# ShenhanQian/GaussianAvatars

Hardware: AMD Instinct MI355X
Metric: frames/sec fwd+bwd @100k SH-3 splats 802x550 (higher is better)
Workload: dtype f32; 1 GPU; BASELINE configs[2]: 100000 mesh-bound SH-3 splats (synthetic stand-in for media/306), 802x550 (HxW), select_mesh_by_timestep + render + L1-vs-white + backward, no optimiser step; splats=100000, width=550, height=802, sh_degree=3, scene=ellipsoid, splat_order=morton (io.spatial_sort: the loaders' default), num_rendered=2322054, num_binned=1851307, tile_culling=True, binding=fused, parallelism=one process, one GPU, 300 frames in turn; no collective

## Files before the change

### gaussianavatars_amd/csrc/gsr_backward.hip

```cpp
#include "gsr_device.h"

#include <hip/amd_detail/amd_hip_unsafe_atomics.h>

namespace gsr {

__device__ __forceinline__ float swap32_add(float a, float b)
{
    const auto r = __builtin_amdgcn_permlane32_swap(__float_as_uint(a), __float_as_uint(b), false, false);
    return __uint_as_float(r[0]) + __uint_as_float(r[1]);
}
__device__ __forceinline__ float swap16_add(float a, float b)
{
    const auto r = __builtin_amdgcn_permlane16_swap(__float_as_uint(a), __float_as_uint(b), false, false);
    return __uint_as_float(r[0]) + __uint_as_float(r[1]);
}
__device__ __forceinline__ float bank_merge(float keep, float take, const int bank_mask_sel)
{
    return bank_mask_sel == 0xA
               ? __int_as_float(__builtin_amdgcn_update_dpp(__float_as_int(keep), __float_as_int(take), 0xE4, 0xf, 0xA, false))
               : __int_as_float(__builtin_amdgcn_update_dpp(__float_as_int(keep), __float_as_int(take), 0xE4, 0xf, 0xC, false));
}
__device__ __forceinline__ float row_sum4(float a, float b, float c, float d)
{
    a += dpp_f<0x141, 0xf>(a);
// ... 354 lines not shown
    const float fqx0 = (float)qx0, fqy0 = (float)qy0;

    for (;;) {
        const int lo = hi - CH;
        const int j = hi - 1 - lane;
        const bool valid = lane < CH && j < nq;
        const uint32_t idx = qp[valid ? j : nq - 1];
        const float4 r0 = grec[3 * (size_t)idx + 0], r1 = grec[3 * (size_t)idx + 1], r2 = grec[3 * (size_t)idx + 2];
        const float xq = r0.x - fqx0, yq = r0.y - fqy0;
        const float cA = r0.z, cB = r0.w, cC = r1.x;
        const float op = valid ? r2.z : 0.f;
        const float cr = r1.z, cgn = r1.w, cb = r2.x;
        const int jrec = valid ? j : 0x7fffffff;
        const unsigned long long act = __ballot(last_pix > lo);
        const bool more = lo > seg_lo;
        f2 a0 = {0.f, 0.f}, a1 = a0, a2 = a0, a3 = a0, a4 = a0, a5 = a0, a6 = a0, a7 = a0, a8 = a0;

        for (int r = 0; r < 8; ++r) {
            const uint32_t rm = (uint32_t)(act >> (8 * r)) & 0xFFu;
            if (!rm) continue;
            const float dy = yq - (float)r;
            const float Bdy = cB * dy, Cdy2 = (cC * dy) * dy;
#ifndef GSR_EXP_NO_ROW_SUMS
            f2 rs0 = {0.f, 0.f}, rs1 = rs0, rs2 = rs0;
#endif
#pragma unroll
            for (int h = 0; h < 2; ++h) {
                if (!((rm >> (4 * h)) & 0xFu)) continue;
                const f4* tp = reinterpret_cast<const f4*>(tab + (r * 4 + 2 * h) * 12);
                f4 t[2][3];
#pragma unroll
                for (int e = 0; e < 2; ++e)
#pragma unroll
                    for (int k = 0; k < 3; ++k) t[e][k] = tp[3 * e + k];
                f2 dx[2], a0m[2], al[2], rv[2], R[2], Tj[2], cg[2], aT[2], Pw[2];
#pragma unroll
                for (int e = 0; e < 2; ++e) {
                    const float c0 = (float)(4 * h + 2 * e);
                    dx[e] = f2{xq - c0, xq - (c0 + 1.0f)};
                    const f2 pw = (cA * dx[e] + Bdy) * dx[e] + Cdy2;
                    const f2 G = {__builtin_amdgcn_exp2f(pw.x), __builtin_amdgcn_exp2f(pw.y)};
                    const f2 araw = op * G;
                    const int l0 = __float_as_int(t[e][2].z), l1 = __float_as_int(t[e][2].w);
#ifdef GSR_EXP_HI_TEST
                    a0m[e].x = (l0 > jrec && pw.x <= 0.0f && araw.x >= 1.0f / 255.0f) ? araw.x : 0.0f;
                    a0m[e].y = (l1 > jrec && pw.y <= 0.0f && araw.y >= 1.0f / 255.0f) ? araw.y : 0.0f;
#else
                    a0m[e].x = (l0 > jrec && araw.x >= 1.0f / 255.0f) ? araw.x : 0.0f;
                    a0m[e].y = (l1 > jrec && araw.y >= 1.0f / 255.0f) ? araw.y : 0.0f;
#endif
                    al[e] = f2{__builtin_fminf(0.99f, a0m[e].x), __builtin_fminf(0.99f, a0m[e].y)};
                    const f2 om = 1.0f - al[e];
                    rv[e] = f2{__builtin_amdgcn_rcpf(om.x), __builtin_amdgcn_rcpf(om.y)};
                    R[e] = rv[e];
                }
#ifndef GSR_EXP_RP_NOSCAN
                GSR_SCAN4("v_mul_f32_dpp", R[0].x, R[0].y, R[1].x, R[1].y);
#endif
#pragma unroll
                for (int e = 0; e < 2; ++e) {
                    const f2 Te = {t[e][0].x, t[e][0].y};
                    const f2 g0 = {t[e][1].x, t[e][1].y}, g1 = {t[e][1].z, t[e][1].w}, g2 = {t[e][2].x, t[e][2].y};
                    Tj[e] = Te * R[e];
                    cg[e] = cr * g0 + (cgn * g1 + cb * g2);
                    aT[e] = al[e] * Tj[e];
                    Pw[e] = aT[e] * cg[e];
                }
#ifndef GSR_EXP_RP_NOSCAN
                GSR_SCAN4("v_add_f32_dpp", Pw[0].x, Pw[0].y, Pw[1].x, Pw[1].y);
#endif
#pragma unroll
                for (int e = 0; e < 2; ++e) {
                    const f2 Sx = {t[e][0].z, t[e][0].w};
                    const f2 g0 = {t[e][1].x, t[e][1].y}, g1 = {t[e][1].z, t[e][1].w}, g2 = {t[e][2].x, t[e][2].y};
                    const f2 dLda = ((Tj[e] * cg[e] - Pw[e]) - Sx) * rv[e];
                    const f2 tq = a0m[e] * dLda;
                    a0 += aT[e] * g0;
                    a1 += aT[e] * g1;
                    a2 += aT[e] * g2;
#ifndef GSR_EXP_NO_ROW_SUMS
                    const f2 ax = tq * dx[e];
                    rs0 += tq;
                    rs1 += ax;
                    rs2 += ax * dx[e];
#else
                    const f2 ax = tq * dx[e], ay = tq * dy;
                    a3 += ax;
                    a4 += ay;
                    a5 += ax * dx[e];
                    a6 += ax * dy;
                    a7 += ay * dy;
                    a8 += tq;
#endif
                    if (more) {
                        const float T0 = __int_as_float(__builtin_amdgcn_readlane(__float_as_int(Tj[e].x), CH - 1));
                        const float T1 = __int_as_float(__builtin_amdgcn_readlane(__float_as_int(Tj[e].y), CH - 1));
                        const float S0 = __int_as_float(__builtin_amdgcn_readlane(__float_as_int(Pw[e].x), CH - 1)) + Sx.x;
                        const float S1 = __int_as_float(__builtin_amdgcn_readlane(__float_as_int(Pw[e].y), CH - 1)) + Sx.y;
                        if (lane == 0) {
                            float* up = tab + (r * 4 + 2 * h + e) * 12;
                            up[0] = T0; up[1] = T1; up[2] = S0; up[3] = S1;
                        }
                    }
                }
            }
#ifndef GSR_EXP_NO_ROW_SUMS
            a3 += rs1;
            a4 += rs0 * dy;
            a5 += rs2;
            a6 += rs1 * dy;
            a7 += rs0 * (dy * dy);
            a8 += rs0;
#endif
        }
#ifndef GSR_EXP_RP_NOATOMIC
        {
            const float v[9] = {a0.x + a0.y, a1.x + a1.y, a2.x + a2.y, a3.x + a3.y, a4.x + a4.y, a5.x + a5.y, a6.x + a6.y, a7.x + a7.y, a8.x + a8.y};
#pragma unroll
            for (int c = 0; c < 9; ++c) xs[9 * lane + c] = v[c];
#pragma unroll
            for (int i = 0; i < (CH + 6) / 7; ++i) {
                const int rl7 = (lane * 7282) >> 16;
                const int c = lane - 9 * rl7;
                const int rl = 7 * i + rl7;
                const float val = xs[63 * i + lane];
                const uint32_t rid = (uint32_t)__builtin_amdgcn_ds_bpermute(rl << 2, (int)idx);
                const bool live = lane < 63 && rl < CH && (hi - 1 - rl) < nq;
#ifdef GSR_EXP_RP_PLAINSTORE
                if (live && val == 12345.678f) acc[(size_t)GSR_ACC_STRIDE * rid + c] = val;
#else
                if (live && val != 0.f) unsafeAtomicAdd(acc + (size_t)GSR_ACC_STRIDE * rid + c, val);
#endif
            }
        }
#endif
        if (!more) break;
        hi = lo;
    }
    }
}

template __global__ void k_render_bwd_rp<1>(Settings, const uint32_t*, const uint32_t*, const float4*, const uint32_t*, const float*, const uint32_t*, const float*, float*, const float*,
                                             const float4*, int, unsigned long long, const unsigned long long*, const uint32_t*);
template __global__ void k_render_bwd_rp<2>(Settings, const uint32_t*, const uint32_t*, const float4*, const uint32_t*, const float*, const uint32_t*, const float*, float*, const float*,
                                             const float4*, int, unsigned long long, const unsigned long long*, const uint32_t*);
template __global__ void k_render_bwd_rp<4>(Settings, const uint32_t*, const uint32_t*, const float4*, const uint32_t*, const float*, const uint32_t*, const float*, float*, const float*,
                                             const float4*, int, unsigned long long, const unsigned long long*, const uint32_t*);


__global__ __launch_bounds__(GSR_PREBWD_ROWS) void k_preprocess_bwd(Settings s, PreBwdArgs a)
{
    const int i = blockIdx.x * blockDim.x + threadIdx.x;
    const int M = a.M;
    __shared__ float sh_lds[GSR_PREBWD_ROWS * GSR_SH_MAX_STRIDE];
    const bool sh_staged = !a.use_precomp_color && a.dL_dsh != nullptr && M <= 16;
    const int first = blockIdx.x * GSR_PREBWD_ROWS, rows = min(GSR_PREBWD_ROWS, a.P - first);
    const int sh_stride = sh_row_stride(M);
    if (sh_staged) {
        if (a.shs_rest) {
            sh_rows_load<GSR_PREBWD_ROWS>(sh_lds, a.shs, first, rows, 3, sh_stride, 0, (int)threadIdx.x);
            sh_rows_load<GSR_PREBWD_ROWS>(sh_lds, a.shs_rest, first, rows, 3 * (M - 1), sh_stride, 3, (int)threadIdx.x);
        } else {
            sh_rows_load<GSR_PREBWD_ROWS>(sh_lds, a.shs, first, rows, 3 * M, sh_stride, 0, (int)threadIdx.x);
        }
        __syncthreads();
    }
    if (i < a.P) {
    float dmean[3] = {0.f, 0.f, 0.f};
    float gcov[6] = {0.f, 0.f, 0.f, 0.f, 0.f, 0.f};
    float dscale[3] = {0.f, 0.f, 0.f};
    float drot[4] = {0.f, 0.f, 0.f, 0.f};
    float gcol[3] = {0.f, 0.f, 0.f};
    float g2x = 0.f, g2y = 0.f, gop = 0.f;
    const bool vis = a.radii[i] > 0;
    float* gsh = a.dL_dsh ? (sh_staged ? sh_lds + (int)threadIdx.x * sh_row_stride(M) : a.dL_dsh + (size_t)3 * M * i) : nullptr;

    if (vis) {
        float4 q0, q1, q2;
        if (s.deterministic) {
            long long* ai = a.acc64 + (size_t)GSR_ACC64_STRIDE * i;
            const int ex = __float_as_int(a.grec[3 * (size_t)i + 2].y), back = gmax_exponent(*a.gmax) - GSR_FIXED_BITS;
            float f[9];
#pragma unroll
            for (int k = 0; k < 9; ++k) { f[k] = __builtin_ldexpf((float)ai[k], back + ((k >= 5 && k <= 7) ? (ex >> 8) : (ex & 0xFF))); ai[k] = 0ll; }
            q0 = make_float4(f[0], f[1], f[2], f[3]); q1 = make_float4(f[4], f[5], f[6], f[7]); q2 = make_float4(f[8], 0.f, 0.f, 0.f);
        } else {
            float4* ac4 = (float4*)(a.acc + (size_t)GSR_ACC_STRIDE * i);
            q0 = ac4[0]; q1 = ac4[1]; q2 = ac4[2];
            const float4 z = make_float4(0.f, 0.f, 0.f, 0.f);
            ac4[0] = z; ac4[1] = z; ac4[2] = z;
        }
        gcol[0] = q0.x; gcol[1] = q0.y; gcol[2] = q0.z;
        g2x = -0.5f * (float)s.W * q0.w; g2y = -0.5f * (float)s.H * q1.x;
        const float gA = -0.5f * q1.y, gB = -0.5f * q1.z, gC = -0.5f * q1.w;
        gop = q2.x;
        const float* vm = s.viewmatrix;
        const float* proj = s.projmatrix;
        const int W = s.W, H = s.H;
        const float fx = (float)W / (2.0f * s.tanfovx), fy = (float)H / (2.0f * s.tanfovy);
        float mx = a.means3D[3 * i], my = a.means3D[3 * i + 1], mz = a.means3D[3 * i + 2];
        if (a.bound.binding) {
            const long long bface = bound_face(a.bound, i);
            float w[3];
            bindm::world_xyz(a.bound.fR + 9 * bface, a.bound.fs[bface], a.bound.fc + 3 * bface, mx, my, mz, w);
            mx = w[0]; my = w[1]; mz = w[2];
        }
        const float* c6 = a.cov3D + 6 * i;

        if (!a.use_precomp_color) {
            float shr[48];
            {
                const float* row = sh_staged ? sh_lds + (int)threadIdx.x * sh_row_stride(M) : a.shs + (size_t)3 * M * i;
#pragma unroll
                for (int k = 0; k < 48; ++k) shr[k] = k < 3 * M ? row[k] : 0.f;
            }
            const float* sh = shr;
            const int deg = s.sh_degree;
            const float d0 = mx - s.campos[0], d1 = my - s.campos[1], d2 = mz - s.campos[2];
            const float sum2 = d0 * d0 + d1 * d1 + d2 * d2;
            const float inv_len = 1.0f / sqrtf(sum2);
            const float x = d0 * inv_len, y = d1 * inv_len, z = d2 * inv_len;
            const uint32_t cl = a.clamped[i];
            float ddir[3] = {0.f, 0.f, 0.f};
            const float xx = x * x, yy = y * y, zz = z * z, xy_ = x * y, yz = y * z, xz = x * z;
            const int ncoef = (deg + 1) * (deg + 1);
#pragma unroll
            for (int c = 0; c < 3; ++c) {
                const float g = ((cl >> c) & 1u) ? 0.f : gcol[c];
                float dxs = 0.f, dys = 0.f, dzs = 0.f;
                gsh[0 + c] = kC0 * g;
                if (deg > 0) {
                    gsh[3 + c] = -kC1 * y * g;
                    gsh[6 + c] = kC1 * z * g;
                    gsh[9 + c] = -kC1 * x * g;
                    dxs = -kC1 * sh[9 + c];
                    dys = -kC1 * sh[3 + c];
                    dzs = kC1 * sh[6 + c];
                    if (deg > 1) {
                        gsh[12 + c] = kC2_0 * xy_ * g;
                        gsh[15 + c] = kC2_1 * yz * g;
                        gsh[18 + c] = kC2_2 * (2.f * zz - xx - yy) * g;
                        gsh[21 + c] = kC2_3 * xz * g;
                        gsh[24 + c] = kC2_4 * (xx - yy) * g;
                        dxs += kC2_0 * y * sh[12 + c] + kC2_2 * 2.f * -x * sh[18 + c] + kC2_3 * z * sh[21 + c] + kC2_4 * 2.f * x * sh[24 + c];
                        dys += kC2_0 * x * sh[12 + c] + kC2_1 * z * sh[15 + c] + kC2_2 * 2.f * -y * sh[18 + c] + kC2_4 * 2.f * -y * sh[24 + c];
                        dzs += kC2_1 * y * sh[15 + c] + kC2_2 * 2.f * 2.f * z * sh[18 + c] + kC2_3 * x * sh[21 + c];
                        if (deg > 2) {
                            gsh[27 + c] = kC3_0 * y * (3.f * xx - yy) * g;
                            gsh[30 + c] = kC3_1 * xy_ * z * g;
                            gsh[33 + c] = kC3_2 * y * (4.f * zz - xx - yy) * g;
                            gsh[36 + c] = kC3_3 * z * (2.f * zz - 3.f * xx - 3.f * yy) * g;
                            gsh[39 + c] = kC3_4 * x * (4.f * zz - xx - yy) * g;
                            gsh[42 + c] = kC3_5 * z * (xx - yy) * g;
                            gsh[45 + c] = kC3_6 * x * (xx - 3.f * yy) * g;
                            dxs += kC3_0 * sh[27 + c] * 3.f * 2.f * xy_ + kC3_1 * sh[30 + c] * yz + kC3_2 * sh[33 + c] * -2.f * xy_ +
                                   kC3_3 * sh[36 + c] * -3.f * 2.f * xz + kC3_4 * sh[39 + c] * (-3.f * xx + 4.f * zz - yy) +
                                   kC3_5 * sh[42 + c] * 2.f * xz + kC3_6 * sh[45 + c] * 3.f * (xx - yy);
                            dys += kC3_0 * sh[27 + c] * 3.f * (xx - yy) + kC3_1 * sh[30 + c] * xz +
                                   kC3_2 * sh[33 + c] * (-3.f * yy + 4.f * zz - xx) + kC3_3 * sh[36 + c] * -3.f * 2.f * yz +
                                   kC3_4 * sh[39 + c] * -2.f * xy_ + kC3_5 * sh[42 + c] * -2.f * yz + kC3_6 * sh[45 + c] * -3.f * 2.f * xy_;
                            dzs += kC3_1 * sh[30 + c] * xy_ + kC3_2 * sh[33 + c] * 4.f * 2.f * yz +
                                   kC3_3 * sh[36 + c] * 3.f * (2.f * zz - xx - yy) + kC3_4 * sh[39 + c] * 4.f * 2.f * xz +
                                   kC3_5 * sh[42 + c] * (xx - yy);
                        }
                    }
                }
                ddir[0] += dxs * g;
                ddir[1] += dys * g;
                ddir[2] += dzs * g;
            }
            for (int k = 3 * ncoef; k < 3 * M; ++k) gsh[k] = 0.f;
            const float invsum32 = 1.0f / sqrtf(sum2 * sum2 * sum2);
            dmean[0] += ((sum2 - d0 * d0) * ddir[0] - d1 * d0 * ddir[1] - d2 * d0 * ddir[2]) * invsum32;
            dmean[1] += (-d0 * d1 * ddir[0] + (sum2 - d1 * d1) * ddir[1] - d2 * d1 * ddir[2]) * invsum32;
            dmean[2] += (-d0 * d2 * ddir[0] - d1 * d2 * ddir[1] + (sum2 - d2 * d2) * ddir[2]) * invsum32;
        }

        float t0 = vm[0] * mx + vm[4] * my + vm[8] * mz + vm[12];
        float t1 = vm[1] * mx + vm[5] * my + vm[9] * mz + vm[13];
        const float t2 = vm[2] * mx + vm[6] * my + vm[10] * mz + vm[14];
        const float limx = 1.3f * s.tanfovx, limy = 1.3f * s.tanfovy;
        const float txtz = t0 / t2, tytz = t1 / t2;
        t0 = sel_min(limx, sel_max(-limx, txtz)) * t2;
        t1 = sel_min(limy, sel_max(-limy, tytz)) * t2;
        const float x_grad_mul = (txtz < -limx || txtz > limx) ? 0.f : 1.f;
        const float y_grad_mul = (tytz < -limy || tytz > limy) ? 0.f : 1.f;
        const float J00 = fx / t2, J02 = -(fx * t0) / (t2 * t2), J11 = fy / t2, J12 = -(fy * t1) / (t2 * t2);
        float A[2][3];
#pragma unroll
        for (int j = 0; j < 3; ++j) {
            A[0][j] = J00 * vm[4 * j + 0] + J02 * vm[4 * j + 2];
            A[1][j] = J11 * vm[4 * j + 1] + J12 * vm[4 * j + 2];
        }
        const float V[3][3] = {{c6[0], c6[1], c6[2]}, {c6[1], c6[3], c6[4]}, {c6[2], c6[4], c6[5]}};
        float AV[2][3];
#pragma unroll
        for (int r = 0; r < 2; ++r)
#pragma unroll
            for (int j = 0; j < 3; ++j) AV[r][j] = A[r][0] * V[0][j] + A[r][1] * V[1][j] + A[r][2] * V[2][j];
        const float ca = AV[0][0] * A[0][0] + AV[0][1] * A[0][1] + AV[0][2] * A[0][2] + 0.3f;
        const float cb = AV[0][0] * A[1][0] + AV[0][1] * A[1][1] + AV[0][2] * A[1][2];
        const float cc = AV[1][0] * A[1][0] + AV[1][1] * A[1][1] + AV[1][2] * A[1][2] + 0.3f;
        const float denom = ca * cc - cb * cb;
        if (s.fast_blend) {
            const float det_inv = 1.f / denom;
            const float kA = cc * det_inv, kB = -cb * det_inv, kC = ca * det_inv;
            g2x = -0.5f * (float)s.W * (kA * q0.w + kB * q1.x);
            g2y = -0.5f * (float)s.H * (kC * q1.x + kB * q0.w);
            const float opac = a.grec[3 * (size_t)i + 2].z;
            gop = opac > 0.f ? q2.x / opac : 0.f;
        }
        const float denom2inv = 1.0f / ((denom * denom) + 0.0000001f);
        float dL_da = 0.f, dL_db = 0.f, dL_dc = 0.f;
        if (denom2inv != 0.f) {
            dL_da = denom2inv * (-cc * cc * gA + 2.f * cb * cc * gB + (denom - ca * cc) * gC);
            dL_dc = denom2inv * (-ca * ca * gC + 2.f * ca * cb * gB + (denom - ca * cc) * gA);
            dL_db = denom2inv * 2.f * (cb * cc * gA - (denom + 2.f * cb * cb) * gB + ca * cb * gC);
            gcov[0] = A[0][0] * A[0][0] * dL_da + A[0][0] * A[1][0] * dL_db + A[1][0] * A[1][0] * dL_dc;
            gcov[3] = A[0][1] * A[0][1] * dL_da + A[0][1] * A[1][1] * dL_db + A[1][1] * A[1][1] * dL_dc;
            gcov[5] = A[0][2] * A[0][2] * dL_da + A[0][2] * A[1][2] * dL_db + A[1][2] * A[1][2] * dL_dc;
            gcov[1] = 2.f * A[0][0] * A[0][1] * dL_da + (A[0][0] * A[1][1] + A[0][1] * A[1][0]) * dL_db + 2.f * A[1][0] * A[1][1] * dL_dc;
            gcov[2] = 2.f * A[0][0] * A[0][2] * dL_da + (A[0][0] * A[1][2] + A[0][2] * A[1][0]) * dL_db + 2.f * A[1][0] * A[1][2] * dL_dc;
            gcov[4] = 2.f * A[0][2] * A[0][1] * dL_da + (A[0][1] * A[1][2] + A[0][2] * A[1][1]) * dL_db + 2.f * A[1][1] * A[1][2] * dL_dc;
        }
        float dA[2][3];
#pragma unroll
        for (int j = 0; j < 3; ++j) {
            const float a0v = A[0][0] * V[j][0] + A[0][1] * V[j][1] + A[0][2] * V[j][2];
            const float a1v = A[1][0] * V[j][0] + A[1][1] * V[j][1] + A[1][2] * V[j][2];
            dA[0][j] = 2.f * a0v * dL_da + a1v * dL_db;
            dA[1][j] = 2.f * a1v * dL_dc + a0v * dL_db;
        }
        const float dJ00 = vm[0] * dA[0][0] + vm[4] * dA[0][1] + vm[8] * dA[0][2];
        const float dJ02 = vm[2] * dA[0][0] + vm[6] * dA[0][1] + vm[10] * dA[0][2];
        const float dJ11 = vm[1] * dA[1][0] + vm[5] * dA[1][1] + vm[9] * dA[1][2];
        const float dJ12 = vm[2] * dA[1][0] + vm[6] * dA[1][1] + vm[10] * dA[1][2];
        const float tz = 1.f / t2, tz2 = tz * tz, tz3 = tz2 * tz;
        const float dtx = x_grad_mul * -fx * tz2 * dJ02;
        const float dty = y_grad_mul * -fy * tz2 * dJ12;
        const float dtz = -fx * tz2 * dJ00 - fy * tz2 * dJ11 + (2.f * fx * t0) * tz3 * dJ02 + (2.f * fy * t1) * tz3 * dJ12;
        dmean[0] += vm[0] * dtx + vm[1] * dty + vm[2] * dtz;
        dmean[1] += vm[4] * dtx + vm[5] * dty + vm[6] * dtz;
        dmean[2] += vm[8] * dtx + vm[9] * dty + vm[10] * dtz;

        const float hw = proj[3] * mx + proj[7] * my + proj[11] * mz + proj[15];
        const float m_w = 1.0f / (hw + 0.0000001f);
        const float mul1 = (proj[0] * mx + proj[4] * my + proj[8] * mz + proj[12]) * m_w * m_w;
        const float mul2 = (proj[1] * mx + proj[5] * my + proj[9] * mz + proj[13]) * m_w * m_w;
        dmean[0] += (proj[0] * m_w - proj[3] * mul1) * g2x + (proj[1] * m_w - proj[3] * mul2) * g2y;
        dmean[1] += (proj[4] * m_w - proj[7] * mul1) * g2x + (proj[5] * m_w - proj[7] * mul2) * g2y;
        dmean[2] += (proj[8] * m_w - proj[11] * mul1) * g2x + (proj[9] * m_w - proj[11] * mul2) * g2y;

        if (!a.use_precomp_cov) {
            float4 q = reinterpret_cast<const float4*>(a.rotations)[i];
            float ws[3] = {a.scales[3 * i], a.scales[3 * i + 1], a.scales[3 * i + 2]};
            if (a.bound.binding) {
                const long long bface = bound_face(a.bound, i);
                q = bindm::world_rotation(reinterpret_cast<const float4*>(a.bound.fq)[bface], q);
                const float bscale = a.bound.fs[bface];
#pragma unroll
                for (int k = 0; k < 3; ++k) ws[k] = bindm::world_scaling(ws[k], bscale);
            } else if (a.bound.leaves) {
                q = bindm::unit_rotation(q);
#pragma unroll
                for (int k = 0; k < 3; ++k) ws[k] = bindm::world_scaling(ws[k], 1.f);
            }
            const float r = q.x, x = q.y, y = q.z, z = q.w;
            float R[3][3];
            R[0][0] = 1.f - 2.f * (y * y + z * z);
            R[0][1] = 2.f * (x * y - r * z);
            R[0][2] = 2.f * (x * z + r * y);
            R[1][0] = 2.f * (x * y + r * z);
            R[1][1] = 1.f - 2.f * (x * x + z * z);
            R[1][2] = 2.f * (y * z - r * x);
            R[2][0] = 2.f * (x * z - r * y);
            R[2][1] = 2.f * (y * z + r * x);
            R[2][2] = 1.f - 2.f * (x * x + y * y);
            const float mod = s.scale_modifier;
            const float sc[3] = {mod * ws[0], mod * ws[1], mod * ws[2]};
            const float gS[3][3] = {{gcov[0], 0.5f * gcov[1], 0.5f * gcov[2]},
                                    {0.5f * gcov[1], gcov[3], 0.5f * gcov[4]},
                                    {0.5f * gcov[2], 0.5f * gcov[4], gcov[5]}};
            float dR[3][3];
#pragma unroll
            for (int k = 0; k < 3; ++k) {
                float dMk[3];
#pragma unroll
                for (int j = 0; j < 3; ++j)
                    dMk[j] = 2.0f * sc[k] * (R[0][k] * gS[0][j] + R[1][k] * gS[1][j] + R[2][k] * gS[2][j]);
                dscale[k] = (s.exact_scale_grad ? mod : 1.0f) * (R[0][k] * dMk[0] + R[1][k] * dMk[1] + R[2][k] * dMk[2]);
#pragma unroll
                for (int j = 0; j < 3; ++j) dR[j][k] = sc[k] * dMk[j];
            }
            drot[0] = 2.f * z * (dR[1][0] - dR[0][1]) + 2.f * y * (dR[0][2] - dR[2][0]) + 2.f * x * (dR[2][1] - dR[1][2]);
            drot[1] = 2.f * y * (dR[0][1] + dR[1][0]) + 2.f * z * (dR[0][2] + dR[2][0]) + 2.f * r * (dR[2][1] - dR[1][2]) - 4.f * x * (dR[2][2] + dR[1][1]);
            drot[2] = 2.f * x * (dR[0][1] + dR[1][0]) + 2.f * r * (dR[0][2] - dR[2][0]) + 2.f * z * (dR[1][2] + dR[2][1]) - 4.f * y * (dR[2][2] + dR[0][0]);
            drot[3] = 2.f * r * (dR[1][0] - dR[0][1]) + 2.f * x * (dR[0][2] + dR[2][0]) + 2.f * y * (dR[1][2] + dR[2][1]) - 4.f * z * (dR[1][1] + dR[0][0]);
        }
    } else if (gsh) {
        for (int k = 0; k < 3 * M; ++k) gsh[k] = 0.f;
    }

    if (a.bound.binding) {
        const long long bface = bound_face(a.bound, i);
        float Rf[9];
#pragma unroll
        for (int k = 0; k < 9; ++k) Rf[k] = a.bound.fR[9 * bface + k];
        const float xl[3] = {a.means3D[3 * i], a.means3D[3 * i + 1], a.means3D[3 * i + 2]};
        const float ls[3] = {a.scales ? a.scales[3 * i] : 0.f, a.scales ? a.scales[3 * i + 1] : 0.f, a.scales ? a.scales[3 * i + 2] : 0.f};
        const float4 ql = a.rotations ? reinterpret_cast<const float4*>(a.rotations)[i] : make_float4(1.f, 0.f, 0.f, 0.f);
        float dx[3], dls[3], acc[BINDM_ROW];
        float4 dq;
        bindm::bind_backward(Rf, a.bound.fs[bface], reinterpret_cast<const float4*>(a.bound.fq)[bface], xl, ls, ql, dmean, dscale,
                             make_float4(drot[0], drot[1], drot[2], drot[3]), dx, dls, &dq, acc);
#pragma unroll
        for (int k = 0; k < 3; ++k) { dmean[k] = dx[k]; dscale[k] = dls[k]; }
        drot[0] = dq.x; drot[1] = dq.y; drot[2] = dq.z; drot[3] = dq.w;
        const float o = bindm::sigmoid(a.opacities[i]);
        gop = gop * o * (1.f - o);
        float4* row = reinterpret_cast<float4*>(a.bound.rows + (size_t)BINDM_ROW * a.bound.slot[i]);
#pragma unroll
        for (int k = 0; k < BINDM_ROW / 4; ++k) row[k] = make_float4(acc[4 * k], acc[4 * k + 1], acc[4 * k + 2], acc[4 * k + 3]);
    }
    else if (a.bound.leaves) {
        if (a.scales) {
#pragma unroll
            for (int k = 0; k < 3; ++k) dscale[k] *= bindm::world_scaling(a.scales[3 * i + k], 1.f);
        }
        if (a.rotations) {
            const float4 dq = bindm::unit_rotation_backward(reinterpret_cast<const float4*>(a.rotations)[i], make_float4(drot[0], drot[1], drot[2], drot[3]));
            drot[0] = dq.x; drot[1] = dq.y; drot[2] = dq.z; drot[3] = dq.w;
        }
        const float o = bindm::sigmoid(a.opacities[i]);
        gop = gop * o * (1.f - o);
    }
#pragma unroll
    for (int k = 0; k < 3; ++k) a.dL_dmeans3D[3 * i + k] = dmean[k];
    a.dL_dmeans2D[3 * i + 0] = g2x;
    a.dL_dmeans2D[3 * i + 1] = g2y;
    a.dL_dmeans2D[3 * i + 2] = 0.f;
    if (a.dL_dcolors) {
#pragma unroll
        for (int k = 0; k < 3; ++k) a.dL_dcolors[3 * i + k] = gcol[k];
    }
    a.dL_dopacity[i] = gop;
    if (a.dL_dcov3D) {
#pragma unroll
        for (int k = 0; k < 6; ++k) a.dL_dcov3D[6 * i + k] = gcov[k];
    }
    if (a.dL_dscales) {
#pragma unroll
        for (int k = 0; k < 3; ++k) a.dL_dscales[3 * i + k] = dscale[k];
    }
    if (a.dL_drotations) reinterpret_cast<float4*>(a.dL_drotations)[i] = make_float4(drot[0], drot[1], drot[2], drot[3]);
    }
    if (sh_staged) {
        __syncthreads();
        if (a.shs_rest) {
            sh_rows_store<GSR_PREBWD_ROWS>(sh_lds, a.dL_dsh, first, rows, 3, sh_stride, 0, (int)threadIdx.x);
            sh_rows_store<GSR_PREBWD_ROWS>(sh_lds, a.dL_dsh_rest, first, rows, 3 * (M - 1), sh_stride, 3, (int)threadIdx.x);
        } else {
            sh_rows_store<GSR_PREBWD_ROWS>(sh_lds, a.dL_dsh, first, rows, 3 * M, sh_stride, 0, (int)threadIdx.x);
        }
    }
}

}
```

### gaussianavatars_amd/csrc/gsr_device.h

```cpp
#pragma once
#include <hip/hip_runtime.h>
#include <stdint.h>

#include "../../include/gsr.h"

#define GSR_WAVE 64
#define GSR_TILE_PIX (GSR_BLOCK_X * GSR_BLOCK_Y)
#define GSR_SORT_LDS_KEYS 8192
#define GSR_SORT_XL_KEYS 16384
#define GSR_SORT_SMALL_KEYS 2048
#define GSR_ACC_STRIDE 16
#define GSR_ACC64_STRIDE 10
#define GSR_FIXED_BITS 58
#define GSR_LDS_HIST_TILES 40960
#define GSR_RANK_MAX_BUCKETS 4096
#define GSR_RANK_HIST_TILES (GSR_LDS_HIST_TILES - GSR_RANK_MAX_BUCKETS)
#define GSR_RANK_BANDS 24
#define GSR_RANK_MAX_BANDS 32
#define GSR_RANK_BAND_CHUNK 256
#define GSR_RANK_IDX_BITS 28
#define GSR_RANK_MAX_SPLATS 262144
#define GSR_RANK_TILE_THREADS 512
#define GSR_RANK_WINDOW 4096
#ifndef GSR_RANK_GROUP
// ... 145 lines not shown
    r.px = px; r.py = py; r.A = A; r.B = B; r.C = C;
    r.tau = 0.f; r.nBiC = 0.f; r.nBiA = 0.f;
    if (!(opacity * 255.0f >= 1.0f)) { r.mode = 2; return r; }
    r.tau = logf(255.0f * opacity) * 1.0001f + 1e-3f;
    if (!(A > 0.f && C > 0.f && (A * C - B * B) > 0.f)) { r.mode = 1; return r; }
    r.nBiC = -B / C;
    r.nBiA = -B / A;
    r.mode = 0;
    return r;
}
__device__ __forceinline__ bool rect_reach(const Reach& r, float x0, float y0, float w, float h)
{
    if (r.mode) return r.mode == 1;
    const float a0 = r.px - (x0 + w), a1 = r.px - x0;
    const float b0 = r.py - (y0 + h), b1 = r.py - y0;
    const bool in_x = a0 <= 0.f && a1 >= 0.f, in_y = b0 <= 0.f && b1 >= 0.f;
    if (in_x && in_y) return true;
    const float a = a0 > 0.f ? a0 : a1;
    const float b = b0 > 0.f ? b0 : b1;
    const float dyv = fminf(fmaxf(r.nBiC * a, b0), b1);
    const float qv = 0.5f * (r.A * a * a + 2.f * r.B * a * dyv + r.C * dyv * dyv);
    const float dxh = fminf(fmaxf(r.nBiA * b, a0), a1);
    const float qh = 0.5f * (r.A * dxh * dxh + 2.f * r.B * dxh * b + r.C * b * b);
    const float big = 3.0e38f;
    const float mn = fminf(in_x ? big : qv, in_y ? big : qh);
    return mn * 0.999f - 1e-3f <= r.tau;
}

struct Span {
    float px, py, B, det, twoTA, A, dyr;
    int mode;
};
__device__ __forceinline__ Span span_of(const Reach& r)
{
    Span s;
    s.px = r.px; s.py = r.py; s.B = r.B; s.mode = r.mode;
    s.det = 0.f; s.twoTA = 0.f; s.A = 0.f; s.dyr = 0.f;
    if (r.mode) return s;
    const float T = (r.tau + 1e-3f) / 0.999f;
    s.det = r.A * r.C - r.B * r.B;
    s.twoTA = 2.f * T * r.A;
    s.A = r.A;
    s.dyr = r.nBiC * sqrtf(2.f * T * r.C / s.det);
    if (!(fabsf(s.dyr) < 1e15f && s.twoTA < 1e30f && s.A > 1e-30f && s.A < 1e30f && s.det > 0.f)) s.mode = 1;
    return s;
}
struct Band {
    float dl, dr, Bbl, Bbr;
    int any;
};
__device__ __forceinline__ Band band_of(const Span& s, float y0)
{
    Band e;
    e.dl = e.dr = e.Bbl = e.Bbr = 0.f;
    if (s.mode) { e.any = s.mode == 1 ? 2 : 0; return e; }
    const float b0 = y0 - s.py, b1 = b0 + 7.f;
    const float br = fminf(fmaxf(s.dyr, b0), b1), bl = fminf(fmaxf(-s.dyr, b0), b1);
    e.dr = s.twoTA - s.det * br * br;
    e.dl = s.twoTA - s.det * bl * bl;
    e.Bbr = s.B * br;
    e.Bbl = s.B * bl;
    e.any = (e.dr >= 0.f && e.dl >= 0.f) ? 1 : 0;
    return e;
}
__device__ __forceinline__ bool band_hit(const Band& e, const Span& s, float x0)
{
    const float tl = (s.px - 1e-2f - (x0 + 7.f)) * s.A - e.Bbl;
    const float tr = (x0 - s.px - 1e-2f) * s.A + e.Bbr;
    const bool hit = (tl <= 0.f || e.dl >= tl * tl) && (tr <= 0.f || e.dr >= tr * tr);
    return e.any == 2 || (e.any == 1 && hit);
}

__device__ __forceinline__ void snug_rect(const Reach& r, int& minx, int& miny, int& maxx, int& maxy, uint32_t& n)
{
    if (r.mode == 1 || n == 0) return;
    if (r.mode == 2) { n = 0; return; }
    const float det = r.A * r.C - r.B * r.B;
    const float k = 2.f * r.tau / det;
    const float xr = sqrtf(k * r.C) * 1.001f + 1e-2f, yr = sqrtf(k * r.A) * 1.001f + 1e-2f;
    if (!(xr < 1e9f && yr < 1e9f)) return;
    const float fx = (float)GSR_BLOCK_X, fy = (float)GSR_BLOCK_Y;
    const int lox = (int)ceilf((r.px - xr - (fx - 1.f)) / fx), hix = (int)floorf((r.px + xr) / fx) + 1;
    const int loy = (int)ceilf((r.py - yr - (fy - 1.f)) / fy), hiy = (int)floorf((r.py + yr) / fy) + 1;
    minx = max(minx, lox); maxx = min(maxx, hix);
    miny = max(miny, loy); maxy = min(maxy, hiy);
    n = (maxx > minx && maxy > miny) ? (uint32_t)((maxx - minx) * (maxy - miny)) : 0u;
}

__device__ __forceinline__ uint32_t quadrant_mask_of(const Span& s, float ox, float oy)
{
    uint32_t m = 0u;
#pragma unroll
    for (int by = 0; by < 2; ++by) {
        const float y0 = by ? oy + 8.f : oy;
        const float b0 = y0 - s.py, b1 = b0 + 7.f;
        const float br = fminf(fmaxf(s.dyr, b0), b1), bl = fminf(fmaxf(-s.dyr, b0), b1);
        const float dr = s.twoTA - s.det * br * br;
        const float dl = s.twoTA - s.det * bl * bl;
        const float Bbr = s.B * br;
        const float Bbl = s.B * bl;
        const uint32_t any = (uint32_t)(dr >= 0.f) & (uint32_t)(dl >= 0.f);
#pragma unroll
        for (int bx = 0; bx < 2; ++bx) {
            const float x0 = bx ? ox + 8.f : ox;
            const float tl = (s.px - 1e-2f - (x0 + 7.f)) * s.A - Bbl;
            const float tr = (x0 - s.px - 1e-2f) * s.A + Bbr;
            const uint32_t hit = ((uint32_t)(tl <= 0.f) | (uint32_t)(dl >= tl * tl)) & ((uint32_t)(tr <= 0.f) | (uint32_t)(dr >= tr * tr)) & any;
            m |= hit << (2 * by + bx);
        }
    }
    return s.mode == 1 ? 15u : (s.mode == 2 ? 0u : m);
}
__device__ __forceinline__ uint32_t quadrant_mask(float2 p, float4 co, float ox, float oy)
{
    return quadrant_mask_of(span_of(reach_of(p.x, p.y, co.x, co.y, co.z, co.w)), ox, oy);
}

template <typename F>
__device__ __forceinline__ void for_each_tile(int minx, int miny, int maxx, int maxy, uint32_t n, int gx, F f,
                                              uint32_t payload0, uint32_t payload1)
{
    constexpr uint32_t SMALL = 16;
    if (n > 0 && n <= SMALL) {
        for (int y = miny; y < maxy; ++y)
            for (int x = minx; x < maxx; ++x) f((uint32_t)(y * gx + x), payload0, payload1);
    }
    uint64_t big = __ballot(n > SMALL);
    const int lane = lane_id();
    while (big) {
        const int src = __builtin_ctzll(big);
        big &= big - 1;
        const int bminx = __builtin_amdgcn_readlane(minx, src);
        const int bminy = __builtin_amdgcn_readlane(miny, src);
        const int bmaxx = __builtin_amdgcn_readlane(maxx, src);
        const uint32_t bn = (uint32_t)__builtin_amdgcn_readlane((int)n, src);
        const uint32_t p0 = (uint32_t)__builtin_amdgcn_readlane((int)payload0, src);
        const uint32_t p1 = (uint32_t)__builtin_amdgcn_readlane((int)payload1, src);
        const uint32_t w = (uint32_t)(bmaxx - bminx);
        for (uint32_t k = (uint32_t)lane; k < bn; k += GSR_WAVE) {
            const uint32_t y = (uint32_t)bminy + k / w;
            const uint32_t x = (uint32_t)bminx + k % w;
            f(y * (uint32_t)gx + x, p0, p1);
        }
    }
}

#define GSR_SH_ROWS 256
#ifndef GSR_PREBWD_ROWS
#define GSR_PREBWD_ROWS 208
#endif
#define GSR_SH_MAX_STRIDE 49
__device__ __forceinline__ int sh_row_stride(int M) { return (3 * M) | 1; }

template <int NT = GSR_SH_ROWS>
__device__ __forceinline__ void sh_rows_load(float* __restrict__ lds, const float* __restrict__ src, int first, int rows, int w, int stride,
                                             int col0, int tid)
{
    const int total = rows * w;
    const float* base = src + (size_t)first * w;
    if ((total & 3) == 0 && ((((size_t)first * w) & 3) == 0)) {
        const float4* b4 = reinterpret_cast<const float4*>(base);
        for (int f = tid * 4; f < total; f += NT * 4) {
            const float4 v = b4[f >> 2];
            int r = f / w, c = f - r * w;
            const float e[4] = {v.x, v.y, v.z, v.w};
#pragma unroll
            for (int k = 0; k < 4; ++k) {
                lds[r * stride + col0 + c] = e[k];
                if (++c == w) { c = 0; ++r; }
            }
        }
    } else {
        for (int f = tid; f < total; f += NT) {
            const int r = f / w, c = f - r * w;
            lds[r * stride + col0 + c] = base[f];
        }
    }
}

template <int NT = GSR_SH_ROWS>
__device__ __forceinline__ void sh_rows_store(const float* __restrict__ lds, float* __restrict__ dst, int first, int rows, int w, int stride,
                                              int col0, int tid)
{
    const int total = rows * w;
    float* base = dst + (size_t)first * w;
    if ((total & 3) == 0 && ((((size_t)first * w) & 3) == 0)) {
        float4* b4 = reinterpret_cast<float4*>(base);
        for (int f = tid * 4; f < total; f += NT * 4) {
            int r = f / w, c = f - r * w;
            float e[4];
#pragma unroll
            for (int k = 0; k < 4; ++k) {
                e[k] = lds[r * stride + col0 + c];
                if (++c == w) { c = 0; ++r; }
            }
            b4[f >> 2] = make_float4(e[0], e[1], e[2], e[3]);
        }
    } else {
        for (int f = tid; f < total; f += NT) {
            const int r = f / w, c = f - r * w;
            base[f] = lds[r * stride + col0 + c];
        }
    }
}

#define GSR_STAT_SLOTS 32
struct BinStatSlot {
    uint32_t nvis, dmin_inv, dmax_bits, pad0;
    unsigned long long binned_tiles, rect_total;
    uint32_t pad1[8];
};
struct BinHeader {
    unsigned long long total;
    unsigned long long rect_total;
    uint32_t nvis;
    uint32_t dmin_inv;
    uint32_t dmax_bits;
    uint32_t dmin_bits;
    unsigned long long binned_tiles;
    uint32_t band_total[GSR_RANK_MAX_BANDS];
    uint32_t chunk_imbalance;
    uint32_t pad[21];
    BinStatSlot slot[GSR_STAT_SLOTS];
};
static_assert(sizeof(BinHeader) == 256 + 64 * GSR_STAT_SLOTS, "header layout is part of include/gsr.h");

#define GSR_WALK_MASKS 2
struct QBinArgs {
    int Q, gx;
    uint32_t chunks;
    BinHeader* __restrict__ hdr;
    const float4* __restrict__ brec;
    const uint32_t* __restrict__ order;
    uint32_t* __restrict__ qhist;
    const uint32_t* __restrict__ qprefix;
    const uint32_t* __restrict__ qstart;
    uint32_t* __restrict__ qpos;
    unsigned long long* __restrict__ qmask;
    unsigned long long capacity;
};

struct BoundDev {
    int leaves;
    const void* __restrict__ binding;
    int is64;
    const float* __restrict__ fR;
    const float* __restrict__ fs;
    const float* __restrict__ fc;
    const float* __restrict__ fq;
    const int* __restrict__ slot;
    float* __restrict__ rows;
};
__device__ __forceinline__ long long bound_face(const BoundDev& b, int i)
{
    return b.is64 ? reinterpret_cast<const long long*>(b.binding)[i] : (long long)reinterpret_cast<const int*>(b.binding)[i];
}

struct PreprocessArgs {
    int P, M;
    const float* __restrict__ means3D;
    const float* __restrict__ shs;
    const float* __restrict__ shs_rest;
    const float* __restrict__ colors_precomp;
    const float* __restrict__ opacities;
    const float* __restrict__ scales;
    const float* __restrict__ rotations;
    const float* __restrict__ cov3D_precomp;
    int32_t* __restrict__ radii;
    float* __restrict__ depths;
    float4* __restrict__ grec;
    float* __restrict__ cov3D;
    ushort4* __restrict__ rect;
    uint32_t* __restrict__ tiles_touched;
    uint8_t* __restrict__ clamped;
    uint8_t* __restrict__ visible;
    float4* __restrict__ acc;
    float4* __restrict__ acc64;
    uint32_t* __restrict__ tile_count;
    uint32_t* __restrict__ units;
    unsigned long long* __restrict__ rect_total;
    int tiles;
    float4* __restrict__ brec;
    BinHeader* __restrict__ hdr;
    uint32_t* __restrict__ bcount;
    int nb;
    uint32_t* __restrict__ bcursor;
    uint4* __restrict__ pstat;
    ushort4* __restrict__ srect;
    float4* __restrict__ sspan;
    int cull;
    BoundDev bound;
};

struct PreBwdArgs {
    int P, M;
    const float* __restrict__ means3D;
    const float* __restrict__ shs;
    const float* __restrict__ shs_rest;
    const float* __restrict__ scales;
    const float* __restrict__ rotations;
    const float* __restrict__ cov3D;
    const int32_t* __restrict__ radii;
    const uint8_t* __restrict__ clamped;
    float* __restrict__ acc;
    long long* __restrict__ acc64;
    const uint32_t* __restrict__ gmax;
    const float4* __restrict__ grec;
    int use_precomp_cov, use_precomp_color;
    float* __restrict__ dL_dmeans3D;
    float* __restrict__ dL_dmeans2D;
    float* __restrict__ dL_dsh;
    float* __restrict__ dL_dsh_rest;
    float* __restrict__ dL_dcolors;
    float* __restrict__ dL_dopacity;
    float* __restrict__ dL_dscales;
    float* __restrict__ dL_drotations;
    float* __restrict__ dL_dcov3D;
    BoundDev bound;
    const float* __restrict__ opacities;
};

__global__ void k_preprocess(Settings s, PreprocessArgs a);
__global__ void k_tile_scan(int tiles, const uint32_t* tile_count, uint32_t* tile_start, uint32_t* tile_cursor, uint2* ranges,
                            uint32_t* tile_order, unsigned long long* total_dev, unsigned long long* mailbox, unsigned long long seq, unsigned long long post_capacity);
template <bool CULL>
__global__ void k_count(int P, int gx, int tiles, const ushort4* rect, const uint32_t* tiles_touched, const float4* grec, uint32_t* tile_count,
                        unsigned long long* rect_total, uint32_t* block_hist);
template <bool CULL>
__global__ void k_scatter(int P, int gx, int tiles, const float* depths, const ushort4* rect, const uint32_t* tiles_touched, const float4* grec,
                          const uint32_t* tile_start, uint32_t* tile_cursor, unsigned long long* keys,
                          unsigned long long capacity, const unsigned long long* total_dev, const uint32_t* block_hist);
// ... 131 lines not shown
```

Baseline: 3841 frames/s.

## Hoist per-splat loads ahead of SH staging and coalesce gradient stores via LDS

The preprocess backward kernel now issues every per-splat global load (accumulators, means, covariance, binding face data, rotation, scale, opacity, slot) at kernel entry, before the SH rows are staged into LDS. The SH staging is split into a request phase that keeps float4 loads in registers and a later land phase, so the loads overlap the face-data fetches. The 3-wide per-splat outputs (dmean, means2D grad, dscale, color grad) are written through LDS and emitted as coalesced float4 stores. The aim is to hide memory latency and avoid strided scalar stores, at the cost of higher register pressure, clamped speculative loads for out-of-range threads, and extra barriers.

```diff
diff --git a/gaussianavatars_amd/csrc/gsr_backward.hip b/gaussianavatars_amd/csrc/gsr_backward.hip
--- a/gaussianavatars_amd/csrc/gsr_backward.hip
+++ b/gaussianavatars_amd/csrc/gsr_backward.hip
@@ -530,41 +530,74 @@
 {
     const int i = blockIdx.x * blockDim.x + threadIdx.x;
     const int M = a.M;
-    __shared__ float sh_lds[GSR_PREBWD_ROWS * GSR_SH_MAX_STRIDE];
+    const int ic = min(i, a.P - 1);
+    const bool bound = a.bound.binding != nullptr;
+    const int* bp = reinterpret_cast<const int*>(bound ? a.bound.binding : (const void*)a.radii);
+    const int b_lo = bp[a.bound.is64 && bound ? 2 * (size_t)ic : (size_t)ic], b_hi = bp[a.bound.is64 && bound ? 2 * (size_t)ic + 1 : (size_t)ic];
+    const int radius = a.radii[ic];
+    const float4* ac4r = reinterpret_cast<const float4*>(s.deterministic ? reinterpret_cast<const char*>(a.acc64) : reinterpret_cast<const char*>(a.acc)) +
+                         (size_t)(GSR_ACC_STRIDE / 4) * ic;
+    float4 q0 = ac4r[0], q1 = ac4r[1], q2 = ac4r[2];
+    const float lm[3] = {a.means3D[3 * ic], a.means3D[3 * ic + 1], a.means3D[3 * ic + 2]};
+    const float2* cv = reinterpret_cast<const float2*>(a.cov3D + 6 * (size_t)ic);
+    const float2 cv0 = cv[0], cv1 = cv[1], cv2 = cv[2];
+    const uint32_t cl = (uint32_t)a.clamped[ic];
+    const float4 rec2 = a.grec[3 * (size_t)ic + 2];
+    const float4 ql_raw = *reinterpret_cast<const float4*>(a.rotations ? a.rotations + 4 * (size_t)ic : a.cov3D);
+    const float* lsp = a.scales ? a.scales + 3 * (size_t)ic : a.cov3D;
+    const float ls_raw[3] = {lsp[0], lsp[1], lsp[2]};
+    const float logit = (bound || a.bound.leaves) ? a.opacities[ic] : 0.f;
+    const int slot = (bound ? a.bound.slot : a.radii)[ic];
+    __shared__ __align__(16) float sh_lds[GSR_PREBWD_ROWS * GSR_SH_MAX_STRIDE];
     const bool sh_staged = !a.use_precomp_color && a.dL_dsh != nullptr && M <= 16;
     const int first = blockIdx.x * GSR_PREBWD_ROWS, rows = min(GSR_PREBWD_ROWS, a.P - first);
     const int sh_stride = sh_row_stride(M);
+    const bool sh_split = a.shs_rest != nullptr;
+    ShRowsInFlight<GSR_PREBWD_ROWS, 1> sh_dc;
+    ShRowsInFlight<GSR_PREBWD_ROWS, 12> sh_main;
     if (sh_staged) {
-        if (a.shs_rest) {
-            sh_rows_load<GSR_PREBWD_ROWS>(sh_lds, a.shs, first, rows, 3, sh_stride, 0, (int)threadIdx.x);
-            sh_rows_load<GSR_PREBWD_ROWS>(sh_lds, a.shs_rest, first, rows, 3 * (M - 1), sh_stride, 3, (int)threadIdx.x);
-        } else {
-            sh_rows_load<GSR_PREBWD_ROWS>(sh_lds, a.shs, first, rows, 3 * M, sh_stride, 0, (int)threadIdx.x);
-        }
+        if (sh_split) sh_dc.request(a.shs, first, rows, 3, (int)threadIdx.x);
+        sh_main.request(sh_split ? a.shs_rest : a.shs, first, rows, sh_split ? 3 * (M - 1) : 3 * M, (int)threadIdx.x);
+    }
+    const long long bface = bound ? (a.bound.is64 ? (long long)(((unsigned long long)(uint32_t)b_hi << 32) | (uint32_t)b_lo) : (long long)b_lo) : 0ll;
+    float Rf[9] = {0.f, 0.f, 0.f, 0.f, 0.f, 0.f, 0.f, 0.f, 0.f}, fcen[3] = {0.f, 0.f, 0.f}, fscale = 0.f;
+    float4 fquat = make_float4(1.f, 0.f, 0.f, 0.f);
+    if (bound) {
+#pragma unroll
+        for (int k = 0; k < 9; ++k) Rf[k] = a.bound.fR[9 * bface + k];
+        fscale = a.bound.fs[bface];
+#pragma unroll
+        for (int k = 0; k < 3; ++k) fcen[k] = a.bound.fc[3 * bface + k];
+        fquat = reinterpret_cast<const float4*>(a.bound.fq)[bface];
+    }
+    if (sh_staged) {
+        if (sh_split) sh_dc.land(sh_lds, a.shs, first, rows, 3, sh_stride, 0, (int)threadIdx.x);
+        sh_main.land(sh_lds, sh_split ? a.shs_rest : a.shs, first, rows, sh_split ? 3 * (M - 1) : 3 * M, sh_stride, sh_split ? 3 : 0, (int)threadIdx.x);
         __syncthreads();
     }
-    if (i < a.P) {
+    const float c6[6] = {cv0.x, cv0.y, cv1.x, cv1.y, cv2.x, cv2.y};
+    const float4 ql = a.rotations ? ql_raw : make_float4(1.f, 0.f, 0.f, 0.f);
+    const float ls[3] = {a.scales ? ls_raw[0] : 0.f, a.scales ? ls_raw[1] : 0.f, a.scales ? ls_raw[2] : 0.f};
     float dmean[3] = {0.f, 0.f, 0.f};
     float gcov[6] = {0.f, 0.f, 0.f, 0.f, 0.f, 0.f};
     float dscale[3] = {0.f, 0.f, 0.f};
     float drot[4] = {0.f, 0.f, 0.f, 0.f};
     float gcol[3] = {0.f, 0.f, 0.f};
     float g2x = 0.f, g2y = 0.f, gop = 0.f;
-    const bool vis = a.radii[i] > 0;
+    if (i < a.P) {
+    const bool vis = radius > 0;
     float* gsh = a.dL_dsh ? (sh_staged ? sh_lds + (int)threadIdx.x * sh_row_stride(M) : a.dL_dsh + (size_t)3 * M * i) : nullptr;
 
     if (vis) {
-        float4 q0, q1, q2;
         if (s.deterministic) {
             long long* ai = a.acc64 + (size_t)GSR_ACC64_STRIDE * i;
-            const int ex = __float_as_int(a.grec[3 * (size_t)i + 2].y), back = gmax_exponent(*a.gmax) - GSR_FIXED_BITS;
+            const int ex = __float_as_int(rec2.y), back = gmax_exponent(*a.gmax) - GSR_FIXED_BITS;
             float f[9];
 #pragma unroll
             for (int k = 0; k < 9; ++k) { f[k] = __builtin_ldexpf((float)ai[k], back + ((k >= 5 && k <= 7) ? (ex >> 8) : (ex & 0xFF))); ai[k] = 0ll; }
             q0 = make_float4(f[0], f[1], f[2], f[3]); q1 = make_float4(f[4], f[5], f[6], f[7]); q2 = make_float4(f[8], 0.f, 0.f, 0.f);
         } else {
             float4* ac4 = (float4*)(a.acc + (size_t)GSR_ACC_STRIDE * i);
-            q0 = ac4[0]; q1 = ac4[1]; q2 = ac4[2];
             const float4 z = make_float4(0.f, 0.f, 0.f, 0.f);
             ac4[0] = z; ac4[1] = z; ac4[2] = z;
         }
@@ -576,14 +609,12 @@
         const float* proj = s.projmatrix;
         const int W = s.W, H = s.H;
         const float fx = (float)W / (2.0f * s.tanfovx), fy = (float)H / (2.0f * s.tanfovy);
-        float mx = a.means3D[3 * i], my = a.means3D[3 * i + 1], mz = a.means3D[3 * i + 2];
-        if (a.bound.binding) {
-            const long long bface = bound_face(a.bound, i);
+        float mx = lm[0], my = lm[1], mz = lm[2];
+        if (bound) {
             float w[3];
-            bindm::world_xyz(a.bound.fR + 9 * bface, a.bound.fs[bface], a.bound.fc + 3 * bface, mx, my, mz, w);
+            bindm::world_xyz(Rf, fscale, fcen, mx, my, mz, w);
             mx = w[0]; my = w[1]; mz = w[2];
         }
-        const float* c6 = a.cov3D + 6 * i;
 
         if (!a.use_precomp_color) {
             float shr[48];
@@ -598,7 +629,6 @@
             const float sum2 = d0 * d0 + d1 * d1 + d2 * d2;
             const float inv_len = 1.0f / sqrtf(sum2);
             const float x = d0 * inv_len, y = d1 * inv_len, z = d2 * inv_len;
-            const uint32_t cl = a.clamped[i];
             float ddir[3] = {0.f, 0.f, 0.f};
             const float xx = x * x, yy = y * y, zz = z * z, xy_ = x * y, yz = y * z, xz = x * z;
             const int ncoef = (deg + 1) * (deg + 1);
@@ -685,7 +715,7 @@
             const float kA = cc * det_inv, kB = -cb * det_inv, kC = ca * det_inv;
             g2x = -0.5f * (float)s.W * (kA * q0.w + kB * q1.x);
             g2y = -0.5f * (float)s.H * (kC * q1.x + kB * q0.w);
-            const float opac = a.grec[3 * (size_t)i + 2].z;
+            const float opac = rec2.z;
             gop = opac > 0.f ? q2.x / opac : 0.f;
         }
         const float denom2inv = 1.0f / ((denom * denom) + 0.0000001f);
@@ -730,12 +760,11 @@
         dmean[2] += (proj[8] * m_w - proj[11] * mul1) * g2x + (proj[9] * m_w - proj[11] * mul2) * g2y;
 
         if (!a.use_precomp_cov) {
-            float4 q = reinterpret_cast<const float4*>(a.rotations)[i];
-            float ws[3] = {a.scales[3 * i], a.scales[3 * i + 1], a.scales[3 * i + 2]};
-            if (a.bound.binding) {
-                const long long bface = bound_face(a.bound, i);
-                q = bindm::world_rotation(reinterpret_cast<const float4*>(a.bound.fq)[bface], q);
-                const float bscale = a.bound.fs[bface];
+            float4 q = ql;
+            float ws[3] = {ls[0], ls[1], ls[2]};
+            if (bound) {
+                q = bindm::world_rotation(fquat, q);
+                const float bscale = fscale;
 #pragma unroll
                 for (int k = 0; k < 3; ++k) ws[k] = bindm::world_scaling(ws[k], bscale);
             } else if (a.bound.leaves) {
@@ -779,56 +808,36 @@
         for (int k = 0; k < 3 * M; ++k) gsh[k] = 0.f;
     }
 
-    if (a.bound.binding) {
-        const long long bface = bound_face(a.bound, i);
-        float Rf[9];
-#pragma unroll
-        for (int k = 0; k < 9; ++k) Rf[k] = a.bound.fR[9 * bface + k];
-        const float xl[3] = {a.means3D[3 * i], a.means3D[3 * i + 1], a.means3D[3 * i + 2]};
-        const float ls[3] = {a.scales ? a.scales[3 * i] : 0.f, a.scales ? a.scales[3 * i + 1] : 0.f, a.scales ? a.scales[3 * i + 2] : 0.f};
-        const float4 ql = a.rotations ? reinterpret_cast<const float4*>(a.rotations)[i] : make_float4(1.f, 0.f, 0.f, 0.f);
+    if (bound) {
         float dx[3], dls[3], acc[BINDM_ROW];
         float4 dq;
-        bindm::bind_backward(Rf, a.bound.fs[bface], reinterpret_cast<const float4*>(a.bound.fq)[bface], xl, ls, ql, dmean, dscale,
+        bindm::bind_backward(Rf, fscale, fquat, lm, ls, ql, dmean, dscale,
                              make_float4(drot[0], drot[1], drot[2], drot[3]), dx, dls, &dq, acc);
 #pragma unroll
         for (int k = 0; k < 3; ++k) { dmean[k] = dx[k]; dscale[k] = dls[k]; }
         drot[0] = dq.x; drot[1] = dq.y; drot[2] = dq.z; drot[3] = dq.w;
-        const float o = bindm::sigmoid(a.opacities[i]);
+        const float o = bindm::sigmoid(logit);
         gop = gop * o * (1.f - o);
-        float4* row = reinterpret_cast<float4*>(a.bound.rows + (size_t)BINDM_ROW * a.bound.slot[i]);
+        float4* row = reinterpret_cast<float4*>(a.bound.rows + (size_t)BINDM_ROW * slot);
 #pragma unroll
         for (int k = 0; k < BINDM_ROW / 4; ++k) row[k] = make_float4(acc[4 * k], acc[4 * k + 1], acc[4 * k + 2], acc[4 * k + 3]);
     }
     else if (a.bound.leaves) {
         if (a.scales) {
 #pragma unroll
-            for (int k = 0; k < 3; ++k) dscale[k] *= bindm::world_scaling(a.scales[3 * i + k], 1.f);
+            for (int k = 0; k < 3; ++k) dscale[k] *= bindm::world_scaling(ls[k], 1.f);
         }
         if (a.rotations) {
-            const float4 dq = bindm::unit_rotation_backward(reinterpret_cast<const float4*>(a.rotations)[i], make_float4(drot[0], drot[1], drot[2], drot[3]));
+            const float4 dq = bindm::unit_rotation_backward(ql, make_float4(drot[0], drot[1], drot[2], drot[3]));
             drot[0] = dq.x; drot[1] = dq.y; drot[2] = dq.z; drot[3] = dq.w;
         }
-        const float o = bindm::sigmoid(a.opacities[i]);
+        const float o = bindm::sigmoid(logit);
         gop = gop * o * (1.f - o);
-    }
-#pragma unroll
-    for (int k = 0; k < 3; ++k) a.dL_dmeans3D[3 * i + k] = dmean[k];
-    a.dL_dmeans2D[3 * i + 0] = g2x;
-    a.dL_dmeans2D[3 * i + 1] = g2y;
-    a.dL_dmeans2D[3 * i + 2] = 0.f;
-    if (a.dL_dcolors) {
-#pragma unroll
-        for (int k = 0; k < 3; ++k) a.dL_dcolors[3 * i + k] = gcol[k];
     }
     a.dL_dopacity[i] = gop;
     if (a.dL_dcov3D) {
 #pragma unroll
         for (int k = 0; k < 6; ++k) a.dL_dcov3D[6 * i + k] = gcov[k];
-    }
-    if (a.dL_dscales) {
-#pragma unroll
-        for (int k = 0; k < 3; ++k) a.dL_dscales[3 * i + k] = dscale[k];
     }
     if (a.dL_drotations) reinterpret_cast<float4*>(a.dL_drotations)[i] = make_float4(drot[0], drot[1], drot[2], drot[3]);
     }
@@ -840,7 +849,32 @@
         } else {
             sh_rows_store<GSR_PREBWD_ROWS>(sh_lds, a.dL_dsh, first, rows, 3 * M, sh_stride, 0, (int)threadIdx.x);
         }
-    }
-}
-
-}
+        __syncthreads();
+    }
+    {
+        const int tix = (int)threadIdx.x;
+        float* const st = sh_lds;
+        const float g2[3] = {g2x, g2y, 0.f};
+#pragma unroll
+        for (int k = 0; k < 3; ++k) {
+            st[3 * tix + k] = dmean[k];
+            st[3 * GSR_PREBWD_ROWS + 3 * tix + k] = g2[k];
+            st[6 * GSR_PREBWD_ROWS + 3 * tix + k] = dscale[k];
+            st[9 * GSR_PREBWD_ROWS + 3 * tix + k] = gcol[k];
+        }
+        __syncthreads();
+        float* const dst[4] = {a.dL_dmeans3D, a.dL_dmeans2D, a.dL_dscales, a.dL_dcolors};
+        const int total = 3 * rows;
+#pragma unroll
+        for (int r = 0; r < 4; ++r) {
+            if (!dst[r]) continue;
+            float* out = dst[r] + (size_t)3 * first;
+            const float* src = st + 3 * GSR_PREBWD_ROWS * r;
+            if (4 * tix + 4 <= total) reinterpret_cast<float4*>(out)[tix] = reinterpret_cast<const float4*>(src)[tix];
+            else if (4 * tix < total)
+                for (int e = 4 * tix; e < total; ++e) out[e] = src[e];
+        }
+    }
+}
+
+}
diff --git a/gaussianavatars_amd/csrc/gsr_device.h b/gaussianavatars_amd/csrc/gsr_device.h
--- a/gaussianavatars_amd/csrc/gsr_device.h
+++ b/gaussianavatars_amd/csrc/gsr_device.h
@@ -321,31 +321,43 @@
 #define GSR_SH_MAX_STRIDE 49
 __device__ __forceinline__ int sh_row_stride(int M) { return (3 * M) | 1; }
 
-template <int NT = GSR_SH_ROWS>
-__device__ __forceinline__ void sh_rows_load(float* __restrict__ lds, const float* __restrict__ src, int first, int rows, int w, int stride,
-                                             int col0, int tid)
-{
-    const int total = rows * w;
-    const float* base = src + (size_t)first * w;
-    if ((total & 3) == 0 && ((((size_t)first * w) & 3) == 0)) {
-        const float4* b4 = reinterpret_cast<const float4*>(base);
-        for (int f = tid * 4; f < total; f += NT * 4) {
-            const float4 v = b4[f >> 2];
-            int r = f / w, c = f - r * w;
-            const float e[4] = {v.x, v.y, v.z, v.w};
+template <int NT, int B>
+struct ShRowsInFlight {
+    static_assert(NT % 4 == 0, "the workgroup's piece of the stream must start on a float4");
+    float4 v[B];
+    __device__ __forceinline__ void request(const float* __restrict__ src, int first, int rows, int w, int tid)
+    {
+        const int n4 = (rows * w) >> 2;
+        const float4* b4 = reinterpret_cast<const float4*>(src + (size_t)first * w);
 #pragma unroll
-            for (int k = 0; k < 4; ++k) {
-                lds[r * stride + col0 + c] = e[k];
-                if (++c == w) { c = 0; ++r; }
+        for (int k = 0; k < B; ++k) {
+            const int f = tid + NT * k;
+            if (f < n4) v[k] = b4[f];
+        }
+    }
+    __device__ __forceinline__ void land(float* __restrict__ lds, const float* __restrict__ src, int first, int rows, int w, int stride, int col0, int tid) const
+    {
+        const int total = rows * w, n4 = total >> 2;
+#pragma unroll
+        for (int k = 0; k < B; ++k) {
+            const int f = tid + NT * k;
+            if (f < n4) {
+                int r = (4 * f) / w, c = 4 * f - r * w;
+                const float e[4] = {v[k].x, v[k].y, v[k].z, v[k].w};
+#pragma unroll
+                for (int j = 0; j < 4; ++j) {
+                    lds[r * stride + col0 + c] = e[j];
+                    if (++c == w) { c = 0; ++r; }
+                }
             }
         }
-    } else {
-        for (int f = tid; f < total; f += NT) {
+        const float* base = src + (size_t)first * w;
+        for (int f = 4 * n4 + tid; f < total; f += NT) {
             const int r = f / w, c = f - r * w;
             lds[r * stride + col0 + c] = base[f];
         }
     }
-}
+};
 
 template <int NT = GSR_SH_ROWS>
 __device__ __forceinline__ void sh_rows_store(const float* __restrict__ lds, float* __restrict__ dst, int first, int rows, int w, int stride,
```

Result: no change. 3809 frames/s (-0.9%).
